# danijar/crafter

Measured on NVIDIA H100. Metric: env_steps_per_sec_random_policy, higher is better.
Workload: dtype int32/f64

## Files before the change

### crafter_b200/csrc/cr_kernels.h

```cpp
#pragma once
#include "cr_common.h"
#include "cr_geom.h"
#include "cr_noise.h"
#include "cr_render.h"
#include "cr_update.h"
#include "cr_worldgen.h"

#ifdef CR_SIMT
#define CR_DYN_SMEM(name) unsigned char *name = simt::dyn_smem()
#else
#define CR_DYN_SMEM(name) extern __shared__ __align__(16) unsigned char name[]
#endif

namespace cr {
namespace kernels {

#ifndef CR_UPDATE_WPB
#define CR_UPDATE_WPB 4
#endif
constexpr int UPDATE_WPB = CR_UPDATE_WPB;
constexpr int SEED_WPB = 4;
constexpr int RENDER_THREADS = RENDER_NT;
#ifndef CR_RENDER_MIN_CTAS
#define CR_RENDER_MIN_CTAS (RENDER_NT <= 128 ? 8 : DEF ? 4 : 2)
#endif
#ifndef CR_WG_THREADS
#define CR_WG_THREADS 256
#endif
#ifndef CR_WG_MIN_CTAS
#define CR_WG_MIN_CTAS 4
#endif
constexpr int WG_THREADS = CR_WG_THREADS;
#ifndef CR_OBJ_THREADS
#define CR_OBJ_THREADS 1024
#endif
constexpr int OBJ_THREADS = CR_OBJ_THREADS;
constexpr int INSTALL_THREADS = 256;

__host__ __device__ inline size_t align16(size_t v) { return (v + 15) & ~(size_t)15; }

__host__ __device__ inline size_t render_tile_offset(const Geom &g) {
  return align16(sizeof(RenderShared)) +
         (g.tile_cache ? align16((size_t)(N_TILES + 1) * g.ux * g.uy * sizeof(uint32_t)) : 16);
}

__host__ __device__ inline size_t update_smem_per_warp(const Geom &g) {
  return align16(sizeof(PlayerS)) + align16(sizeof(Ent) * ENT_SMEM) + align16(sizeof(uint32_t) * g.TW);
}

template <bool DEF>
__global__ void __launch_bounds__(UPDATE_WPB * 32)
k_update(Geom g, State st, const double *__restrict__ daylight, const int32_t *__restrict__ actions,
         float *reward, uint8_t *done, int auto_reset, int debug_skip) {
  geom_specialize<DEF>(g);
  CR_DYN_SMEM(smem);
  const int warp = threadIdx.x >> 5, lane = threadIdx.x & 31;
  const int env = blockIdx.x * UPDATE_WPB + warp;
  if (env >= g.B) return;
  unsigned char *base = smem + warp * update_smem_per_warp(g);
  PlayerS *P = reinterpret_cast<PlayerS *>(base);
  Ent *sents = reinterpret_cast<Ent *>(base + align16(sizeof(PlayerS)));
  uint32_t *stouched = reinterpret_cast<uint32_t *>(
      base + align16(sizeof(PlayerS)) + align16(sizeof(Ent) * ENT_SMEM));
  int action = actions[env];
  if (action < 0 || action >= N_ACTIONS) action = ACT_NOOP;
  const int kind = env_step(g, st, daylight, env, lane, action, P, sents, stouched, reward, done, auto_reset,
// ... 238 lines not shown
    wg_install_clear_rows(g, st, env, cx * CHUNK, imin(cx * CHUNK + CHUNK, g.W), threadIdx.x, INSTALL_THREADS);
    if (cx == 0)
      for (int c = threadIdx.x; c < g.TW; c += INSTALL_THREADS) st.touched[(size_t)env * g.TW + c] = 0;
    __syncthreads();
    if (g.incr_census)
      census_recount_column(g, st.mat + (size_t)env * g.NC, st.chunk_cnt + (size_t)env * g.NCH * 2, cx, threadIdx.x,
                            INSTALL_THREADS);
  }
}
template <bool DEF>
__global__ void __launch_bounds__(INSTALL_THREADS) k_install(Geom g, State st) {
  geom_specialize<DEF>(g);
  const int count = *st.reset_count;
  if (threadIdx.x == 0 && blockIdx.x < 1023) cr_stamp(4096 + (int)blockIdx.x, 4);
  for (int r = blockIdx.x; r < count; r += gridDim.x) {
    const int env = st.reset_list[r];
    wg_install_scatter(g, st, env, threadIdx.x, INSTALL_THREADS);
    if (threadIdx.x == 0) wg_install_player(g, st, env);
    __syncthreads();
  }
  if (threadIdx.x == 0 && blockIdx.x < 1023) cr_stamp(4096 + (int)blockIdx.x, 5);
}

__device__ __forceinline__ void store_tile(uint8_t *out, uint8_t *tile, size_t bytes, int tid, int evict_first) {
#ifndef CR_SIMT
  if ((bytes & 15) == 0) {
    asm volatile("fence.proxy.async.shared::cta;" ::: "memory");
    __syncthreads();
    if (tid == 0) {
      uint32_t saddr = (uint32_t)__cvta_generic_to_shared(tile);
      if (evict_first) {
        uint64_t policy;
        asm volatile("createpolicy.fractional.L2::evict_first.b64 %0, 1.0;" : "=l"(policy));
        asm volatile("cp.async.bulk.global.shared::cta.bulk_group.L2::cache_hint [%0], [%1], %2, %3;"
                     :: "l"(out), "r"(saddr), "r"((uint32_t)bytes), "l"(policy) : "memory");
      } else
      asm volatile("cp.async.bulk.global.shared::cta.bulk_group [%0], [%1], %2;"
                   :: "l"(out), "r"(saddr), "r"((uint32_t)bytes) : "memory");
      asm volatile("cp.async.bulk.commit_group;" ::: "memory");
      asm volatile("cp.async.bulk.wait_group.read 0;" ::: "memory");
    }
    return;
  }
#endif
  __syncthreads();
  for (size_t i = tid; i < bytes; i += RENDER_THREADS) out[i] = tile[i];
}

__global__ void __launch_bounds__(INSTALL_THREADS) k_recount(Geom g, State st) {
  for (int env = blockIdx.x; env < g.B; env += gridDim.x) {
    __syncthreads();
    census_recount(g, st.mat + (size_t)env * g.NC, st.chunk_cnt + (size_t)env * g.NCH * 2, threadIdx.x,
                   INSTALL_THREADS);
  }
}

template <bool DEF>
__device__ __forceinline__ void render_env(const Geom &g, const State &st, const RenderTables &rt, int env,
                                           uint8_t *out, int staged, unsigned char *smem, int tid, int use_view = 0) {
  RenderShared &S = *reinterpret_cast<RenderShared *>(smem);
  uint32_t *tiles = reinterpret_cast<uint32_t *>(smem + align16(sizeof(RenderShared)));
  uint8_t *tile = smem + render_tile_offset(g);
  const int trow = (tid & 31) == 0 && tid < 64 && env < 4096 ? (3 + (tid >> 5)) * 4096 + env : 1 << 30;
  cr_stamp(trow, 0);
  const int32_t *ps = st.pstate + (size_t)env * PS_COUNT;
  const double daylight = rt.daylight[imin(ps[PS_STEP], g.n_daylight - 1)];
  const size_t bytes = (size_t)g.sw * g.sh * 3;
  const RenderView *ahead = use_view ? reinterpret_cast<const RenderView *>(st.frame_view) + env : nullptr;
  render_stage(g, st, rt, env, tid, RENDER_THREADS, S, daylight, ahead, st.frame_night + env);
  cr_stamp(trow, 1);
  __syncthreads();
  cr_stamp(trow, 2);
  render_tiles(g, rt, S, tiles, tid, RENDER_THREADS, daylight < 0.5, ps[PS_SLEEPING]);
  cr_stamp(trow, 3);
  __syncthreads();
  cr_stamp(trow, 4);
  if (!DEF && !staged) {
    render_assemble(g, st, rt, S, tiles, env, tid, RENDER_THREADS, out, daylight, (bytes & 3) == 0);
    return;
  }
  render_assemble(g, st, rt, S, tiles, env, tid, RENDER_THREADS, tile, daylight, true, true);
  cr_stamp(trow, 5);
  store_tile(out, tile, bytes, tid, g.obs_evict_first);
  cr_stamp(trow, 6);
  cr_stamp(trow, 7, (daylight < 0.5 ? 1000 : 0) + S.V.n_jobs);
}

template <bool DEF>
__global__ void __launch_bounds__(RENDER_THREADS, CR_RENDER_MIN_CTAS)
k_render(Geom g, State st, RenderTables rt, uint8_t *__restrict__ obs, int staged,
         const int32_t *__restrict__ env_list, int out_by_env, int use_view) {
  geom_specialize<DEF>(g);
  CR_DYN_SMEM(smem);
  const int env = env_list ? env_list[blockIdx.x] : (int)blockIdx.x;
  const int row = out_by_env ? env : (int)blockIdx.x;
  render_env<DEF>(g, st, rt, env, obs + (size_t)row * g.sw * g.sh * 3, staged, smem, threadIdx.x, use_view);
}

constexpr int VIEW_WPB = 4;
template <bool DEF>
__global__ void __launch_bounds__(VIEW_WPB * 32) k_view(Geom g, State st, RenderTables rt) {
  geom_specialize<DEF>(g);
  __shared__ RenderView sv[VIEW_WPB];
  const int warp = threadIdx.x >> 5, lane = threadIdx.x & 31;
  const int env = blockIdx.x * VIEW_WPB + warp;
  if (threadIdx.x == 0 && blockIdx.x < 1024) cr_stamp(4096 + 3072 + (int)blockIdx.x, 0);
  if (env >= g.B || !(st.frame_night[env] & FRAME_FINAL)) return;
  RenderView &V = sv[warp];
  render_gather(g, st, rt, env, lane, V);
  __syncwarp();
  const Word16 *src = reinterpret_cast<const Word16 *>(&V);
  Word16 *dst = reinterpret_cast<Word16 *>(st.frame_view) + (size_t)env * VIEW_WORDS;
  for (int i = lane; i < VIEW_WORDS; i += 32) dst[i] = src[i];
  if (lane == 0 && blockIdx.x < 1024) cr_stamp(4096 + 3072 + (int)blockIdx.x, 1 + warp);
}

template <bool DEF>
__global__ void __launch_bounds__(RENDER_THREADS, 3)
k_terminal(Geom g, State st, RenderTables rt) {
// ... 35 lines not shown
```

### crafter_b200/csrc/cr_render.h

```cpp
#pragma once
#include "cr_common.h"

namespace cr {

#ifndef CR_MAX_OBJ_TILES
#define CR_MAX_OBJ_TILES 24
#endif
constexpr int MAX_OBJ_TILES = CR_MAX_OBJ_TILES;
constexpr int TILE_MAT0 = 0, TILE_OBJ0 = 13, TILE_ITEM0 = 13 + MAX_OBJ_TILES;
constexpr int N_TILES = TILE_ITEM0 + N_ITEMS;

struct RenderTables {
  const uint32_t *mat_tex;
  const uint32_t *obj_tex;
  const uint32_t *item_tile;
  const double *vignette;
  const double *daylight;
  const uint16_t *colx;
  const uint16_t *rowy;
};

struct alignas(16) RenderView {
  int32_t inv[N_ITEMS];
  int32_t n_obj, n_jobs, pad0, pad1;
// ... 65 lines not shown
CR_DEV void render_plan(const Geom &g, RenderView &V, int lane);

CR_DEV void render_tables(int tid, int nthreads, RenderShared &S, double daylight) {
  const double inv_d = 1 - daylight;
  for (int v = tid - CR_LANES; v < 256; v += nthreads - CR_LANES) {
    const double dv = (double)v;
    S.D[v] = dv;
    S.A[v] = daylight * dv;
    double half = (1 - 0.5) * dv;
    S.B[0][v] = inv_d * (half + 0.5 * 0.0);
    S.B[1][v] = inv_d * (half + 0.5 * 16.0);
    S.B[2][v] = inv_d * (half + 0.5 * 64.0);
    S.inv255[v] = (float)v / 255.0f;
  }
}

CR_DEV void render_gather(const Geom &g, const State &st, const RenderTables &rt, int env, int lane,
                          RenderView &V);

struct alignas(16) Word16 { uint64_t a, b; };
constexpr int VIEW_WORDS = (int)(sizeof(RenderView) / 16);

CR_DEV void render_stage(const Geom &g, const State &st, const RenderTables &rt, int env, int tid,
                         int nthreads, RenderShared &S, double daylight, const RenderView *ahead = nullptr,
                         const uint8_t *flag = nullptr) {
  if (tid >= CR_LANES) {
    render_tables(tid, nthreads, S, daylight);
  } else if (ahead) {
    constexpr int PER = (VIEW_WORDS + CR_LANES - 1) / CR_LANES;
    const Word16 *src = reinterpret_cast<const Word16 *>(ahead);
    Word16 *dst = reinterpret_cast<Word16 *>(&S.V);
    Word16 w[PER];
#pragma unroll
    for (int q = 0; q < PER; ++q) {
      const int i = tid + q * CR_LANES;
      if (i < VIEW_WORDS) w[q] = src[i];
    }
    if (*flag & FRAME_FINAL) {
#pragma unroll
      for (int q = 0; q < PER; ++q) {
        const int i = tid + q * CR_LANES;
        if (i < VIEW_WORDS) dst[i] = w[q];
      }
    } else {
      render_gather(g, st, rt, env, tid, S.V);
    }
  } else {
    render_gather(g, st, rt, env, tid, S.V);
  }
}

CR_DEV void render_gather(const Geom &g, const State &st, const RenderTables &rt, int env, int lane,
                          RenderView &V) {
  const int32_t *ps = st.pstate + (size_t)env * PS_COUNT;
  const int px = ps[PS_PX], py = ps[PS_PY], sleeping = ps[PS_SLEEPING];
  const uint8_t *mat = st.mat + (size_t)env * g.NC;
  const uint16_t *objmap = st.objmap + (size_t)env * g.NC;
  const Ent *ents = st.ents + (size_t)env * g.CAP;
  const int offx = g.gx / 2, offy = g.gy / 2;
  const int32_t *inv = st.inventory + (size_t)env * N_ITEMS;
  for (int i = lane; i < N_ITEMS; i += CR_LANES) V.inv[i] = inv[i];
  cr_syncwarp();
  constexpr int MAXC = 256 / CR_LANES > 8 ? 256 : 8;
  const int cells = g.vw * g.vh;
  int gcell[MAXC], mm[MAXC], slot[MAXC];
#pragma unroll
  for (int q = 0; q < MAXC; ++q) {
    const int c = lane + q * CR_LANES;
    gcell[q] = -1; mm[q] = 0; slot[q] = 0;
    if (c < cells) {
      const int i = c / g.vh, j = c - i * g.vh;
      const int wx = px + i - offx, wy = py + j - offy;
// ... 55 lines not shown
    }
    n += cr_popc(mask);
  }
  present = cr_reduce_or(present) & 0x1FFFu;
  const int n_mat = cr_popc(present), n_obj = imin(n, MAX_OBJ_TILES);
  for (int m = lane; m < 13; m += CR_LANES)
    if ((present >> m) & 1u) V.job_tile[cr_popc(present & ((1u << m) - 1u))] = (uint8_t)(TILE_MAT0 + m);
  for (int k = lane; k < n_obj; k += CR_LANES) V.job_tile[n_mat + k] = (uint8_t)(TILE_OBJ0 + k);
  int n_item = 0;
  for (int base = 0; base < N_ITEMS; base += CR_LANES) {
    const int i = base + lane;
    const bool has = i < N_ITEMS && V.inv[i] >= 1;
    const uint32_t mask = cr_ballot(has);
    if (has) V.job_tile[n_mat + n_obj + n_item + cr_popc(mask & cr_lanemask_lt(lane))] = (uint8_t)(TILE_ITEM0 + i);
    n_item += cr_popc(mask);
  }
  if (lane == 0) {
    V.job_tile[n_mat + n_obj + n_item] = (uint8_t)N_TILES;
    V.n_obj = n_obj;
    V.n_jobs = n_mat + n_obj + n_item + 1;
  }
}

CR_DEV void render_tiles(const Geom &g, const RenderTables &rt, const RenderShared &S, uint32_t *tiles,
                         int tid, int nthreads, bool dark, int sleeping) {
  const int tsz = g.ux * g.uy;
  const int n_jobs = S.V.n_jobs;
  int t = (int)mulhi32((uint32_t)tid, g.tsz_magic), texel = tid - t * tsz;
  const int sq = g.tile_sq, sr = g.tile_sr;
  (void)nthreads;
  while (t < n_jobs) {
    const int tile = S.V.job_tile[t];
    uint32_t color;
    bool fx = !dark;
    if (tile < TILE_OBJ0) {
      color = rt.mat_tex[tile * tsz + texel] & 0x00FFFFFFu;
    } else if (tile < TILE_ITEM0) {
      const int c = S.V.ocell[tile - TILE_OBJ0];
      color = blend_texel(S, rt.mat_tex[S.V.tmat[c] * tsz + texel], rt.obj_tex[S.V.tobj[c] * tsz + texel]);
    } else if (tile < N_TILES) {
      const int index = tile - TILE_ITEM0;
      int amount = S.V.inv[index];
      if (amount > 9) amount = 0;
      color = rt.item_tile[(index * 10 + amount) * tsz + texel] & 0x00FFFFFFu;
      fx = false;
    } else {
      color = 0;
      fx = false;
    }
    tiles[tile * tsz + texel] = fx ? color_fx(S, color, color, sleeping) : color;
    texel += sr; t += sq;
    if (texel >= tsz) { texel -= tsz; ++t; }
  }
}

struct RenderCtx {
  bool dark;
  int sleeping;
  double amount;
  uint32_t world_seed, step;
};

CR_DEV uint32_t night_pixel_v(const RenderShared &S, const RenderCtx &C, uint32_t c, double vignette,
                              uint32_t w) {
  const double u = (double)(int64_t)(((uint64_t)32 << 32) + (uint64_t)w * 95u) * (1.0 / 4294967296.0);
  const double mask = C.amount * vignette;
  const double om = 1 - mask, mu = mask * u;
  const int n0 = (int)(om * S.D[c & 0xFF] + mu);
  const int n1 = (int)(om * S.D[(c >> 8) & 0xFF] + mu);
  const int n2 = (int)(om * S.D[(c >> 16) & 0xFF] + mu);
  return color_mix3(S, c, n0, n1, n2);
}
CR_DEV uint32_t night_pixel_w(const Geom &g, const RenderTables &rt, const RenderShared &S,
                              const RenderCtx &C, uint32_t c, int cx, int cy, uint32_t w) {
  const uint32_t rgb = night_pixel_v(S, C, c, rt.vignette[cy * g.lw + cx], w);
  return C.sleeping ? sleep_fx(rgb) : rgb;
}
CR_DEV uint32_t night_pixel(const Geom &g, const RenderTables &rt, const RenderShared &S,
                            const RenderCtx &C, uint32_t c, int cx, int cy, U4 &nz, int &nz_block) {
  if ((cx >> 2) != nz_block) {
    nz = philox4x32(C.world_seed, D_NOISE, (uint32_t)(cx >> 2), C.step, (uint32_t)cy, 0);
    nz_block = cx >> 2;
  }
  return night_pixel_w(g, rt, S, C, c, cx, cy, nz.w[cx & 3]);
// ... 20 lines not shown
  } else {
    color = rt.mat_tex[S.V.tmat[cell] * tsz + texel] & 0x00FFFFFFu;
    if (S.V.tobj[cell] != 255) color = blend_texel(S, color, rt.obj_tex[S.V.tobj[cell] * tsz + texel]);
    if (!night) return color_fx(S, color, color, C.sleeping);
  }
  return night_pixel(g, rt, S, C, color, i * g.ux + tx, j * g.uy + ty, nz, nz_block);
}

CR_DEV void store_group(uint8_t *tile_out, int p, const uint32_t *px, int count, bool words_ok) {
  if (words_ok && count == 4) {
    uint32_t *w = (uint32_t *)(tile_out + (size_t)p * 3);
    w[0] = px[0] | (px[1] << 24);
    w[1] = (px[1] >> 8) | (px[2] << 16);
    w[2] = (px[2] >> 16) | (px[3] << 8);
  } else {
    for (int k = 0; k < count; ++k) {
      tile_out[(size_t)(p + k) * 3 + 0] = (uint8_t)px[k];
      tile_out[(size_t)(p + k) * 3 + 1] = (uint8_t)(px[k] >> 8);
      tile_out[(size_t)(p + k) * 3 + 2] = (uint8_t)(px[k] >> 16);
    }
  }
}

CR_DEV void render_assemble(const Geom &g, const State &st, const RenderTables &rt,
                            const RenderShared &S, const uint32_t *tiles, int env, int tid,
                            int nthreads, uint8_t *out, double daylight, bool words_ok, bool out_shared = false) {
  const int32_t *ps = st.pstate + (size_t)env * PS_COUNT;
  RenderCtx C;
  C.dark = daylight < 0.5;
  C.sleeping = ps[PS_SLEEPING];
  C.amount = 2 * (0.5 - daylight);
  C.world_seed = (uint32_t)ps[PS_WORLD_SEED];
  C.step = (uint32_t)ps[PS_STEP];
  const int tsz = g.ux * g.uy;
  if (g.g4_log2 >= 0 && nthreads == RENDER_NT && g.tile_cache) {
    const int gcol = tid & ((1 << g.g4_log2) - 1), band = tid >> g.g4_log2;
    const int y0 = band * g.band_rows, y1 = imin(g.sh, y0 + g.band_rows);
    const int black = N_TILES * tsz;
    int ci[4], toff[4], cx[4];
    bool colok[4];
#pragma unroll
    for (int k = 0; k < 4; ++k) {
      const uint32_t cxi = rt.colx[gcol * 4 + k];
      colok[k] = cxi != 0xFFFFu;
      ci[k] = colok[k] ? (int)(cxi >> 8) * g.vh : -1;
      toff[k] = colok[k] ? (int)(cxi & 0xFF) * g.uy : 0;
      cx[k] = colok[k] ? (int)(cxi >> 8) * g.ux + (int)(cxi & 0xFF) : 0;
    }
    const bool aligned4 = (g.bx & 3) == 0;
    const int out0 = gcol * 4;
    const bool any_col = colok[0] || colok[1] || colok[2] || colok[3];
#define CR_ROW_STATE()                   \
    int cur_j = -1, base[4] = {black, black, black, black};                                  \
    bool slow = false;
#define CR_ROW_LOOKUP()                                                                      \
        const int j = ryi >> 8, ty = ryi & 0xFF;                                             \
// ... 130 lines not shown
#undef CR_DAY_ROWS
#undef CR_NIGHT_ROWS
#undef CR_NIGHT_GROUP
#undef CR_DAY_RUNS
#undef CR_ROW_LOOKUP
#undef CR_ROW_SLOW
#undef CR_PIXEL
#undef CR_ROW_STORE
  } else {
    const int G = (g.sw + 3) >> 2;
    for (int q = tid; q < G * g.sh; q += nthreads) {
      const int y = q / G, x0 = (q - y * G) * 4;
      const uint32_t ryi = rt.rowy[y];
      const int count = imin(4, g.sw - x0);
      U4 nz; nz.w[0] = nz.w[1] = nz.w[2] = nz.w[3] = 0;
      int nz_block = -1;
      uint32_t px[4];
      for (int k = 0; k < count; ++k)
        px[k] = render_pixel(g, rt, S, tiles, C, rt.colx[x0 + k], ryi, nz, nz_block);
      store_group(out, y * g.sw + x0, px, count, words_ok && (((size_t)(y * g.sw + x0) * 3) & 3) == 0);
    }
  }
}

CR_DEV uint8_t semantic_cell(const Geom &g, const State &st, int env, int cell) {
  int slot = st.objmap[(size_t)env * g.NC + cell];
  if (slot) return (uint8_t)(12 + st.ents[(size_t)env * g.CAP + slot].type);
  return st.mat[(size_t)env * g.NC + cell] & 0x7F;
}

}
```

### crafter_b200/csrc/crafter_kernels.cu

```cuda
#include <cuda_runtime.h>
#include <stdio.h>
#include <stdlib.h>
#include <string.h>

#include <mutex>

#include "../../include/crafter_b200.h"
#include "cr_common.h"
#include "cr_geom.h"
#include "cr_noise.h"
#include "cr_render.h"
#include "cr_update.h"
#include "cr_worldgen.h"
#include "cr_kernels.h"

using namespace cr;
using namespace cr::kernels;

namespace {

#define CR_LAUNCH(KERNEL, DEFAULT, GRID, BLOCK, SMEM, STREAM, ...)                       \
  do {                                                                                   \
    if (DEFAULT) KERNEL<true><<<GRID, BLOCK, SMEM, STREAM>>>(__VA_ARGS__);               \
    else KERNEL<false><<<GRID, BLOCK, SMEM, STREAM>>>(__VA_ARGS__);                      \
// ... 24 lines not shown
  static int n = 0;
  std::lock_guard<std::mutex> lock(mu);
  int i = 0;
  while (i < n && funcs[i] != func) ++i;
  if (i == n) {
    if (n == 32) return cudaErrorInvalidValue;
    funcs[n] = func; have[n] = 0; ++n;
  }
  if (bytes <= have[i]) return cudaSuccess;
  cudaError_t e = cudaFuncSetAttribute(func, cudaFuncAttributeMaxDynamicSharedMemorySize, (int)bytes);
  if (e == cudaSuccess) have[i] = bytes;
  return e;
}

}

struct GraphSlot {
  cudaGraphExec_t exec;
  const void *actions, *obs, *reward, *done, *reward_host, *done_host;
  int kernels;
};

enum { TK_UPDATE = 0, TK_INSTALL, TK_RENDER, TK_SEED, TK_MAT, TK_OBJ, TK_AHEAD, TK_BALANCE, TK_COUNT };

struct cr_handle {
  int device;
  Geom g;
  State st;
  RenderTables rt;
  int auto_reset;
  int use_graph;
  int num_sms;
  size_t update_smem, render_smem, balance_smem, terminal_smem;
  int balance_threads;
  int render_staged;
  int64_t launches;
  cudaStream_t side, side2, side3;
  cudaEvent_t ev_fork, ev_join, ev_mat, ev_ahead, ev_inst, ev_d2h, ev_post, ev_bal, ev_view;
  int is_default;
  int timing;
  int debug_skip;
  cudaEvent_t t_ev[TK_COUNT][2];
  double t_ms[TK_COUNT];
  int64_t t_n;
  GraphSlot slots[2];
  float *d2h_reward;
  uint8_t *d2h_done;
  int32_t *err_word;
};

namespace {

inline void tmark(cr_handle *h, int id, int end, cudaStream_t s) {
  if (!h->timing) return;
  cudaStreamCaptureStatus cap = cudaStreamCaptureStatusNone;
  cudaStreamIsCapturing(s, &cap);
  if (cap == cudaStreamCaptureStatusActive) cudaEventRecordWithFlags(h->t_ev[id][end], s, cudaEventRecordExternal);
  else cudaEventRecord(h->t_ev[id][end], s);
// ... 36 lines not shown
  CR_LAUNCH(k_wg_mat, h->is_default, mat_grid, WG_THREADS, 0, s, g, h->st, list, count, only_invalid);
  tmark(h, TK_MAT, 1, s);
  int obj_grid = g.B < h->num_sms * 2 ? g.B : h->num_sms * 2;
  tmark(h, TK_OBJ, 0, s);
  CR_LAUNCH(k_wg_obj, h->is_default, obj_grid, OBJ_THREADS, 0, s, g, h->st, list, count, only_invalid);
  tmark(h, TK_OBJ, 1, s);
  if (ahead) CR_CUDA(cudaStreamWaitEvent(s, h->ev_ahead, 0));
  CR_CUDA(cudaGetLastError());
  return n;
}

int launch_install(cr_handle *h, cudaStream_t s) {
  int grid = h->g.B < h->num_sms * 8 ? h->g.B : h->num_sms * 8;
  long long parts = (long long)h->g.B * h->g.ncx;
  int map_grid = (int)(parts < (long long)h->num_sms * 8 ? parts : (long long)h->num_sms * 8);
  tmark(h, TK_INSTALL, 0, s);
  CR_LAUNCH(k_install_map, h->is_default, map_grid, INSTALL_THREADS, 0, s, h->g, h->st);
  CR_LAUNCH(k_install, h->is_default, grid, INSTALL_THREADS, 0, s, h->g, h->st);
  tmark(h, TK_INSTALL, 1, s);
  CR_CUDA(cudaGetLastError());
  return 2;
}

int launch_render(cr_handle *h, uint8_t *obs, cudaStream_t s, const int32_t *env_list = nullptr, int n_envs = -1,
                  int out_by_env = 0, int use_view = 0) {
  tmark(h, TK_RENDER, 0, s);
  CR_LAUNCH(k_render, h->is_default, n_envs < 0 ? h->g.B : n_envs, RENDER_THREADS, h->render_smem, s, h->g,
            h->st, h->rt, obs, h->render_staged, env_list, out_by_env, use_view);
  tmark(h, TK_RENDER, 1, s);
  CR_CUDA(cudaGetLastError());
  return 1;
}
int launch_render_and_prefetch(cr_handle *h, uint8_t *obs, cudaStream_t s, int seeded) {
  CR_CUDA(cudaEventRecord(h->ev_fork, s));
  CR_CUDA(cudaStreamWaitEvent(h->side, h->ev_fork, 0));
  int n = 0, k;
  if (obs) {
    if ((k = launch_render(h, obs, s)) < 0) return k;
    n += k;
  }
  if ((k = launch_worldgen(h, h->side, h->st.reset_list, h->st.reset_count, 0, 1, seeded)) < 0) return k;
  n += k;
  CR_CUDA(cudaEventRecord(h->ev_join, h->side));
  CR_CUDA(cudaStreamWaitEvent(s, h->ev_join, 0));
  return n;
}

int enqueue_d2h(cr_handle *h, const float *reward, const uint8_t *done, cudaStream_t s) {
  CR_CUDA(cudaMemcpyAsync(h->d2h_reward, reward, (size_t)h->g.B * sizeof(float), cudaMemcpyDeviceToHost, s));
  CR_CUDA(cudaMemcpyAsync(h->d2h_done, done, (size_t)h->g.B, cudaMemcpyDeviceToHost, s));
  return 0;
}

int enqueue_step(cr_handle *h, const int32_t *actions, uint8_t *obs, float *reward, uint8_t *done,
                 cudaStream_t s) {
  const Geom &g = h->g;
  const State &st = h->st;
  int n = 0, k;
#ifdef CR_MEMSET_FIRST
  CR_CUDA(cudaMemsetAsync(st.reset_count, 0, sizeof(int32_t), s));
  CR_CUDA(cudaMemsetAsync(st.balance_count, 0, sizeof(int32_t), s));
// ... 27 lines not shown
      n += 1;
    }
    if ((k = launch_install(h, h->side)) < 0) return k;
    n += k;
    CR_CUDA(cudaEventRecord(h->ev_inst, h->side));
    if ((k = launch_worldgen(h, h->side, st.reset_list, st.reset_count, 0, 1, 1)) < 0) return k;
    n += k;
    CR_CUDA(cudaMemsetAsync(st.reset_count, 0, sizeof(int32_t), h->side));
    CR_CUDA(cudaEventRecord(h->ev_join, h->side));
  }
  const int bal_ctas = g.B < h->num_sms * 4 ? g.B : h->num_sms * 4;
  tmark(h, TK_BALANCE, 0, s);
  CR_LAUNCH(k_post, h->is_default, bal_ctas + (st.frame_order ? 1 : 0), h->balance_threads, h->balance_smem, s, g, st,
            h->rt.daylight, bal_ctas);
  tmark(h, TK_BALANCE, 1, s);
  CR_CUDA(cudaGetLastError());
  n += 1;
  CR_CUDA(cudaEventRecord(h->ev_post, s));
  CR_CUDA(cudaStreamWaitEvent(h->side2, h->ev_post, 0));
  CR_CUDA(cudaMemsetAsync(st.balance_count, 0, sizeof(int32_t), h->side2));
  CR_CUDA(cudaEventRecord(h->ev_bal, h->side2));
  if (h->auto_reset) CR_CUDA(cudaStreamWaitEvent(s, h->ev_inst, 0));
  if (st.frame_view) CR_CUDA(cudaStreamWaitEvent(s, h->ev_view, 0));
  if ((k = launch_render(h, obs, s, st.frame_order, -1, 1, st.frame_view != nullptr)) < 0) return k;
  n += k;
  CR_CUDA(cudaStreamWaitEvent(s, h->ev_bal, 0));
  if (h->auto_reset) CR_CUDA(cudaStreamWaitEvent(s, h->ev_join, 0));
  if (d2h) CR_CUDA(cudaStreamWaitEvent(s, h->ev_d2h, 0));
  return n;
}

void destroy_handle(cr_handle *h) {
  if (!h) return;
  for (int i = 0; i < 2; ++i)
    if (h->slots[i].exec) cudaGraphExecDestroy(h->slots[i].exec);
  cudaStream_t streams[] = {h->side, h->side2, h->side3};
  for (cudaStream_t st : streams)
    if (st) { cudaStreamSynchronize(st); cudaStreamDestroy(st); }
  cudaEvent_t evs[] = {h->ev_mat, h->ev_ahead, h->ev_inst, h->ev_d2h, h->ev_fork, h->ev_join, h->ev_post, h->ev_bal,
                       h->ev_view};
  for (cudaEvent_t e : evs)
    if (e) cudaEventDestroy(e);
  for (int i = 0; i < TK_COUNT; ++i)
    for (int j = 0; j < 2; ++j)
      if (h->t_ev[i][j]) cudaEventDestroy(h->t_ev[i][j]);
  if (h->err_word) cudaFree(h->err_word);
  if (h->st.frame_order) cudaFree(h->st.frame_order);
  free(h);
}

bool env_is(const char *name, char c) {
  const char *v = getenv(name);
  return v && v[0] == c;
}

int create_on_device(cr_handle *h, const cr_config *c, const cr_tables *t, const cr_state *s) {
  Geom &g = h->g;
  if (const char *msg = geom_from_config(*c, g)) return fail_msg(msg);
  state_from_abi(*s, h->st);
  h->st.frame_order = nullptr; h->st.frame_night = nullptr; h->st.frame_view = nullptr;
  h->is_default = geom_is_default(g) && !env_is("CRAFTER_B200_NO_SPECIALIZE", '1');
  h->rt.mat_tex = t->mat_tex; h->rt.obj_tex = t->obj_tex; h->rt.item_tile = t->item_tile;
  h->rt.vignette = t->vignette; h->rt.daylight = t->daylight; h->rt.colx = t->colx;
  h->rt.rowy = t->rowy;
  h->auto_reset = c->auto_reset;
  const char *tm = getenv("CRAFTER_B200_TIMING");
  h->timing = tm && (tm[0] == '1' || tm[0] == '2') ? tm[0] - '0' : 0;
  const char *ds = getenv("CRAFTER_B200_DEBUG_SKIP");
  h->debug_skip = ds ? atoi(ds) : 0;
// ... 6 lines not shown
  CR_CUDA(cudaDeviceGetAttribute(&h->num_sms, cudaDevAttrMultiProcessorCount, dev));
  if (!env_is("CRAFTER_B200_FRAME_ORDER", '0')) {
    const size_t head = align16((size_t)g.B * (sizeof(int32_t) + 1));
    const size_t views = env_is("CRAFTER_B200_VIEW_AHEAD", '0') ? 0 : (size_t)g.B * sizeof(RenderView);
    CR_CUDA(cudaMalloc(&h->st.frame_order, head + views));
    CR_CUDA(cudaMemset(h->st.frame_order, 0, head + views));
    h->st.frame_night = reinterpret_cast<uint8_t *>(h->st.frame_order + g.B);
    if (views) h->st.frame_view = reinterpret_cast<unsigned char *>(h->st.frame_order) + head;
  }
  int max_smem = 0;
  CR_CUDA(cudaDeviceGetAttribute(&max_smem, cudaDevAttrMaxSharedMemoryPerBlockOptin, dev));
  h->update_smem = UPDATE_WPB * update_smem_per_warp(g);
  if (h->update_smem > (size_t)max_smem) return fail_msg("view too large for the update window");
  h->balance_smem = balance_smem(g);
  h->balance_threads = g.NCH * 3 > 4 * BALANCE_THREADS ? BALANCE_THREADS_MAX : BALANCE_THREADS;
  if (h->balance_smem > (size_t)max_smem) return fail_msg("area too large for k_balance");
  CR_CUDA(raise_smem((const void *)k_post<true>, h->balance_smem));
  CR_CUDA(raise_smem((const void *)k_post<false>, h->balance_smem));
  const size_t tile = align16((size_t)g.sw * g.sh * 3);
  if (g.tile_cache && render_tile_offset(g) > (size_t)max_smem) g.tile_cache = 0;
  const size_t fixed = render_tile_offset(g);
  if (fixed > (size_t)max_smem) return fail_msg("unit too large for the tile cache");
  h->render_staged = fixed + tile <= (size_t)max_smem / 2;
  h->render_smem = fixed + (h->render_staged ? tile : 0);
  if (!h->render_staged) h->is_default = 0;
  CR_CUDA(raise_smem((const void *)k_render<true>, h->render_smem));
  CR_CUDA(raise_smem((const void *)k_render<false>, h->render_smem));
  CR_CUDA(raise_smem((const void *)k_update<true>, h->update_smem));
  CR_CUDA(raise_smem((const void *)k_update<false>, h->update_smem));
  g.obs_evict_first = !env_is("CRAFTER_B200_OBS_EVICT_FIRST", '0');
  if (h->st.final_obs) {
    h->terminal_smem = terminal_smem(g, h->render_smem);
    if (!h->render_staged || !g.tile_cache || h->terminal_smem > (size_t)max_smem)
      return fail_msg("final_obs needs a frame that fits the shared-memory staging");
    CR_CUDA(raise_smem((const void *)k_terminal<true>, h->terminal_smem));
    CR_CUDA(raise_smem((const void *)k_terminal<false>, h->terminal_smem));
  }
  if (h->timing)
    for (int i = 0; i < TK_COUNT; ++i)
      for (int j = 0; j < 2; ++j) CR_CUDA(cudaEventCreate(&h->t_ev[i][j]));
  CR_CUDA(cudaStreamCreateWithFlags(&h->side, cudaStreamNonBlocking));
  CR_CUDA(cudaStreamCreateWithFlags(&h->side2, cudaStreamNonBlocking));
  CR_CUDA(cudaStreamCreateWithFlags(&h->side3, cudaStreamNonBlocking));
  cudaEvent_t *evs[] = {&h->ev_mat, &h->ev_ahead, &h->ev_inst, &h->ev_d2h, &h->ev_fork, &h->ev_join, &h->ev_post, &h->ev_bal,
                        &h->ev_view};
  for (cudaEvent_t *e : evs) CR_CUDA(cudaEventCreateWithFlags(e, cudaEventDisableTiming));
  return 0;
}

}

struct DeviceGuard {
  int prev = -1;
  explicit DeviceGuard(int want) {
    int cur = want;
// ... 91 lines not shown
                 uint8_t *done_host, int32_t *actions_dev, uint8_t *obs_dev, float *reward_dev,
                 uint8_t *done_dev, void *stream) {
  if (!h || !actions_host || !reward_host || !done_host) return fail_msg("null argument");
  DeviceGuard on_device(h->device);
  cudaStream_t s = (cudaStream_t)stream;
  const size_t B = (size_t)h->g.B;
  CR_CUDA(cudaMemcpyAsync(actions_dev, actions_host, B * sizeof(int32_t), cudaMemcpyHostToDevice, s));
  h->d2h_reward = reward_host;
  h->d2h_done = done_host;
  int rc = cr_step(h, actions_dev, obs_dev, reward_dev, done_dev, stream);
  h->d2h_reward = nullptr;
  h->d2h_done = nullptr;
  if (rc) return rc;
  if (obs_host)
    CR_CUDA(cudaMemcpyAsync(obs_host, obs_dev, B * h->g.sw * h->g.sh * 3, cudaMemcpyDeviceToHost, s));
  CR_CUDA(cudaStreamSynchronize(s));
  return 0;
}

int cr_render(cr_handle *h, uint8_t *obs, void *stream) {
  if (!h || !obs) return fail_msg("null argument");
  DeviceGuard on_device(h->device);
  const bool as_step = h->st.frame_view && env_is("CRAFTER_B200_RENDER_AS_STEP", '1');
  int k = as_step ? launch_render(h, obs, (cudaStream_t)stream, h->st.frame_order, -1, 1, 1)
                  : launch_render(h, obs, (cudaStream_t)stream);
  if (k < 0) return k;
  h->launches += k;
  return 0;
}

int cr_render_envs(cr_handle *h, const int32_t *env_ids, int n, uint8_t *obs, void *stream) {
  if (!h || !obs || !env_ids) return fail_msg("null argument");
  DeviceGuard on_device(h->device);
  if (n < 0 || n > h->g.B) return fail_msg("cr_render_envs: n out of range");
  if (n == 0) return 0;
  int k = launch_render(h, obs, (cudaStream_t)stream, env_ids, n);
  if (k < 0) return k;
  h->launches += k;
  return 0;
}

int cr_semantic(cr_handle *h, uint8_t *out, void *stream) {
  if (!h || !out) return fail_msg("null argument");
  DeviceGuard on_device(h->device);
  size_t n = (size_t)h->g.B * h->g.NC;
  k_semantic<<<(unsigned)((n + 255) / 256), 256, 0, (cudaStream_t)stream>>>(h->g, h->st, out);
  CR_CUDA(cudaGetLastError());
  h->launches += 1;
  return 0;
}

int cr_recount(cr_handle *h, void *stream) {
  if (!h) return fail_msg("null handle");
  if (!h->g.incr_census) return 0;
  DeviceGuard on_device(h->device);
  const int grid = h->g.B < h->num_sms * 8 ? h->g.B : h->num_sms * 8;
  k_recount<<<grid, INSTALL_THREADS, 0, (cudaStream_t)stream>>>(h->g, h->st);
  CR_CUDA(cudaGetLastError());
  h->launches += 1;
// ... 42 lines not shown
```

Measured before the change: 29.86 million.

## Make render kernel persistent with double-buffered staging and prefetched per-frame state

Turns k_render into a persistent kernel sized to resident CTAs that pulls frames from an atomic ticket counter. It prefetches the next frame's env id, player state, daylight and precomputed view with cp.async, and double-buffers the output staging tile so the bulk store of one frame overlaps assembly of the next. It also batches texture loads in render_tiles so several fetches are in flight at once. In exchange it uses more shared memory per CTA, which may cut occupancy, adds ticket atomics and reset logic, and makes the render loop harder to follow.

```diff
diff --git a/crafter_b200/csrc/cr_kernels.h b/crafter_b200/csrc/cr_kernels.h
--- a/crafter_b200/csrc/cr_kernels.h
+++ b/crafter_b200/csrc/cr_kernels.h
@@ -42,6 +42,9 @@
 __host__ __device__ inline size_t render_tile_offset(const Geom &g) {
   return align16(sizeof(RenderShared)) +
          (g.tile_cache ? align16((size_t)(N_TILES + 1) * g.ux * g.uy * sizeof(uint32_t)) : 16);
+}
+__host__ __device__ inline size_t render_smem_of(const Geom &g, int out_bufs) {
+  return render_tile_offset(g) + (size_t)out_bufs * align16((size_t)g.sw * g.sh * 3);
 }
 
 __host__ __device__ inline size_t update_smem_per_warp(const Geom &g) {
@@ -326,7 +329,7 @@
   if (threadIdx.x == 0 && blockIdx.x < 1023) cr_stamp(4096 + (int)blockIdx.x, 5);
 }
 
-__device__ __forceinline__ void store_tile(uint8_t *out, uint8_t *tile, size_t bytes, int tid, int evict_first) {
+__device__ __forceinline__ void store_tile_issue(uint8_t *out, uint8_t *tile, size_t bytes, int tid, int evict_first) {
 #ifndef CR_SIMT
   if ((bytes & 15) == 0) {
     asm volatile("fence.proxy.async.shared::cta;" ::: "memory");
@@ -342,7 +345,6 @@
       asm volatile("cp.async.bulk.global.shared::cta.bulk_group [%0], [%1], %2;"
                    :: "l"(out), "r"(saddr), "r"((uint32_t)bytes) : "memory");
       asm volatile("cp.async.bulk.commit_group;" ::: "memory");
-      asm volatile("cp.async.bulk.wait_group.read 0;" ::: "memory");
     }
     return;
   }
@@ -350,6 +352,32 @@
   __syncthreads();
   for (size_t i = tid; i < bytes; i += RENDER_THREADS) out[i] = tile[i];
 }
+__device__ __forceinline__ void bulk_wait_read(int pending) {
+#ifndef CR_SIMT
+  if (pending == 0) asm volatile("cp.async.bulk.wait_group.read 0;" ::: "memory");
+  else asm volatile("cp.async.bulk.wait_group.read 1;" ::: "memory");
+#else
+  (void)pending;
+#endif
+}
+__device__ __forceinline__ void store_tile(uint8_t *out, uint8_t *tile, size_t bytes, int tid, int evict_first) {
+  store_tile_issue(out, tile, bytes, tid, evict_first);
+  if (tid == 0) bulk_wait_read(0);
+}
+
+#ifdef CR_SIMT
+__device__ __forceinline__ void cr_cp_async4(void *dst, const void *src) { memcpy(dst, src, 4); }
+__device__ __forceinline__ void cr_cp_async16(void *dst, const void *src) { memcpy(dst, src, 16); }
+__device__ __forceinline__ void cr_cp_async_wait() {}
+#else
+__device__ __forceinline__ void cr_cp_async4(void *dst, const void *src) {
+  asm volatile("cp.async.ca.shared.global [%0], [%1], 4;" :: "r"(cr_saddr(dst)), "l"(src) : "memory");
+}
+__device__ __forceinline__ void cr_cp_async16(void *dst, const void *src) {
+  asm volatile("cp.async.cg.shared.global [%0], [%1], 16;" :: "r"(cr_saddr(dst)), "l"(src) : "memory");
+}
+__device__ __forceinline__ void cr_cp_async_wait() { asm volatile("cp.async.wait_all;" ::: "memory"); }
+#endif
 
 __global__ void __launch_bounds__(INSTALL_THREADS) k_recount(Geom g, State st) {
   for (int env = blockIdx.x; env < g.B; env += gridDim.x) {
@@ -361,7 +389,7 @@
 
 template <bool DEF>
 __device__ __forceinline__ void render_env(const Geom &g, const State &st, const RenderTables &rt, int env,
-                                           uint8_t *out, int staged, unsigned char *smem, int tid, int use_view = 0) {
+                                           uint8_t *out, int staged, unsigned char *smem, int tid) {
   RenderShared &S = *reinterpret_cast<RenderShared *>(smem);
   uint32_t *tiles = reinterpret_cast<uint32_t *>(smem + align16(sizeof(RenderShared)));
   uint8_t *tile = smem + render_tile_offset(g);
@@ -370,8 +398,7 @@
   const int32_t *ps = st.pstate + (size_t)env * PS_COUNT;
   const double daylight = rt.daylight[imin(ps[PS_STEP], g.n_daylight - 1)];
   const size_t bytes = (size_t)g.sw * g.sh * 3;
-  const RenderView *ahead = use_view ? reinterpret_cast<const RenderView *>(st.frame_view) + env : nullptr;
-  render_stage(g, st, rt, env, tid, RENDER_THREADS, S, daylight, ahead, st.frame_night + env);
+  render_stage(g, st, rt, env, tid, RENDER_THREADS, S, daylight);
   cr_stamp(trow, 1);
   __syncthreads();
   cr_stamp(trow, 2);
@@ -390,15 +417,120 @@
   cr_stamp(trow, 7, (daylight < 0.5 ? 1000 : 0) + S.V.n_jobs);
 }
 
+struct alignas(16) FrameSlot {
+  int32_t ps[PS_COUNT];
+  int32_t frame, env;
+  uint32_t flags_word;
+  int32_t pad;
+  double daylight;
+  double pad2;
+};
+
 template <bool DEF>
 __global__ void __launch_bounds__(RENDER_THREADS, CR_RENDER_MIN_CTAS)
 k_render(Geom g, State st, RenderTables rt, uint8_t *__restrict__ obs, int staged,
-         const int32_t *__restrict__ env_list, int out_by_env, int use_view) {
+         const int32_t *__restrict__ env_list, int out_by_env, int use_view, int n_frames = -1, int out_bufs = 1,
+         int32_t *ticket = nullptr) {
   geom_specialize<DEF>(g);
   CR_DYN_SMEM(smem);
-  const int env = env_list ? env_list[blockIdx.x] : (int)blockIdx.x;
-  const int row = out_by_env ? env : (int)blockIdx.x;
-  render_env<DEF>(g, st, rt, env, obs + (size_t)row * g.sw * g.sh * 3, staged, smem, threadIdx.x, use_view);
+  __shared__ FrameSlot slots[2];
+  __shared__ RenderView vnext_s;
+  if (n_frames < 0) n_frames = g.B;
+  RenderShared &S = *reinterpret_cast<RenderShared *>(smem);
+  uint32_t *tiles = reinterpret_cast<uint32_t *>(smem + align16(sizeof(RenderShared)));
+  RenderView *vnext = &vnext_s;
+  uint8_t *staging = smem + render_tile_offset(g);
+  const int tid = threadIdx.x, lane = tid & 31;
+  const size_t bytes = (size_t)g.sw * g.sh * 3;
+  auto fetch_env = [&](FrameSlot &F, int frame) {
+    F.frame = frame;
+    if (frame < n_frames) {
+      if (env_list) cr_cp_async4(&F.env, env_list + frame);
+      else F.env = frame;
+    }
+  };
+  auto fetch_state = [&](FrameSlot &F) {
+    if (F.frame >= n_frames) return;
+    const int env = F.env;
+    if (lane < PS_COUNT) cr_cp_async4(&F.ps[lane], st.pstate + (size_t)env * PS_COUNT + lane);
+    if (use_view) {
+      if (lane == PS_COUNT) cr_cp_async4(&F.flags_word, st.frame_night + (env & ~3));
+      const Word16 *src = reinterpret_cast<const Word16 *>(st.frame_view) + (size_t)env * VIEW_WORDS;
+      for (int i = lane; i < VIEW_WORDS; i += 32) cr_cp_async16(reinterpret_cast<Word16 *>(vnext) + i, src + i);
+    }
+  };
+  auto fetch_daylight = [&](FrameSlot &F) {
+    if (F.frame < n_frames) F.daylight = rt.daylight[imin(F.ps[PS_STEP], g.n_daylight - 1)];
+  };
+  if (tid < 32) {
+    if (lane == 0) fetch_env(slots[0], (int)blockIdx.x);
+    cr_cp_async_wait();
+    __syncwarp();
+    fetch_state(slots[0]);
+    cr_cp_async_wait();
+    __syncwarp();
+    if (lane == 0) fetch_daylight(slots[0]);
+  }
+  __syncthreads();
+  int next_frame = 0;
+  for (int k = 0;; ++k) {
+    FrameSlot &F = slots[k & 1], &Fn = slots[(k + 1) & 1];
+    if (F.frame >= n_frames) break;
+    const int env = F.env;
+    const double daylight = F.daylight;
+    uint8_t *out = obs + (size_t)(out_by_env ? env : F.frame) * bytes;
+    const int trow = (tid & 31) == 0 && tid < 64 && env < 4096 ? (3 + (tid >> 5)) * 4096 + env : 1 << 30;
+    cr_stamp(trow, 0);
+    if (tid >= CR_LANES) {
+      render_tables(tid, RENDER_THREADS, S, daylight);
+    } else {
+      if (lane == 0) next_frame = (int)gridDim.x + (ticket ? atomicAdd(ticket, 1) : F.frame);
+      if (use_view && ((F.flags_word >> (8 * (env & 3))) & FRAME_FINAL)) {
+        const Word16 *src = reinterpret_cast<const Word16 *>(vnext);
+        Word16 *dst = reinterpret_cast<Word16 *>(&S.V);
+        for (int i = lane; i < VIEW_WORDS; i += 32) dst[i] = src[i];
+      } else {
+        render_gather(g, st, rt, env, lane, S.V);
+      }
+    }
+    cr_stamp(trow, 1);
+    __syncthreads();
+    cr_stamp(trow, 2);
+    if (tid == 0) fetch_env(Fn, next_frame);
+    render_tiles(g, rt, S, tiles, tid, RENDER_THREADS, daylight < 0.5, F.ps[PS_SLEEPING]);
+    cr_stamp(trow, 3);
+    const bool direct = !DEF && !staged;
+    uint8_t *tile = staging + (size_t)(out_bufs > 1 ? (k & 1) : 0) * align16(bytes);
+    if (tid == 0 && !direct) bulk_wait_read(out_bufs > 1 ? 1 : 0);
+    __syncthreads();
+    cr_stamp(trow, 4);
+    if (tid < 32) {
+      cr_cp_async_wait();
+      __syncwarp();
+      fetch_state(Fn);
+    }
+    const RenderCtx C = render_ctx(F.ps, daylight);
+    render_assemble(g, rt, S, tiles, C, tid, RENDER_THREADS, direct ? out : tile, direct ? (bytes & 3) == 0 : true,
+                    !direct);
+    cr_stamp(trow, 5);
+    cr_stamp(trow, 7, (long long)(blockIdx.x + 1) * 10000 + (daylight < 0.5 ? 1000 : 0) + S.V.n_jobs);
+    if (tid < 32) {
+      cr_cp_async_wait();
+      __syncwarp();
+      if (lane == 0) fetch_daylight(Fn);
+    }
+    if (direct) __syncthreads();
+    else store_tile_issue(out, tile, bytes, tid, g.obs_evict_first);
+    cr_stamp(trow, 6);
+  }
+  if (tid == 0) {
+    bulk_wait_read(0);
+    __threadfence();
+    if (ticket && atomicAdd(ticket + 1, 1) == (int)gridDim.x - 1) {
+      ticket[0] = 0;
+      ticket[1] = 0;
+    }
+  }
 }
 
 constexpr int VIEW_WPB = 4;
diff --git a/crafter_b200/csrc/cr_render.h b/crafter_b200/csrc/cr_render.h
--- a/crafter_b200/csrc/cr_render.h
+++ b/crafter_b200/csrc/cr_render.h
@@ -111,32 +111,9 @@
 constexpr int VIEW_WORDS = (int)(sizeof(RenderView) / 16);
 
 CR_DEV void render_stage(const Geom &g, const State &st, const RenderTables &rt, int env, int tid,
-                         int nthreads, RenderShared &S, double daylight, const RenderView *ahead = nullptr,
-                         const uint8_t *flag = nullptr) {
-  if (tid >= CR_LANES) {
-    render_tables(tid, nthreads, S, daylight);
-  } else if (ahead) {
-    constexpr int PER = (VIEW_WORDS + CR_LANES - 1) / CR_LANES;
-    const Word16 *src = reinterpret_cast<const Word16 *>(ahead);
-    Word16 *dst = reinterpret_cast<Word16 *>(&S.V);
-    Word16 w[PER];
-#pragma unroll
-    for (int q = 0; q < PER; ++q) {
-      const int i = tid + q * CR_LANES;
-      if (i < VIEW_WORDS) w[q] = src[i];
-    }
-    if (*flag & FRAME_FINAL) {
-#pragma unroll
-      for (int q = 0; q < PER; ++q) {
-        const int i = tid + q * CR_LANES;
-        if (i < VIEW_WORDS) dst[i] = w[q];
-      }
-    } else {
-      render_gather(g, st, rt, env, tid, S.V);
-    }
-  } else {
-    render_gather(g, st, rt, env, tid, S.V);
-  }
+                         int nthreads, RenderShared &S, double daylight) {
+  if (tid >= CR_LANES) render_tables(tid, nthreads, S, daylight);
+  else render_gather(g, st, rt, env, tid, S.V);
 }
 
 CR_DEV void render_gather(const Geom &g, const State &st, const RenderTables &rt, int env, int lane,
@@ -238,6 +215,7 @@
   }
 }
 
+constexpr int TILE_BATCH = 4;
 CR_DEV void render_tiles(const Geom &g, const RenderTables &rt, const RenderShared &S, uint32_t *tiles,
                          int tid, int nthreads, bool dark, int sleeping) {
   const int tsz = g.ux * g.uy;
@@ -246,27 +224,46 @@
   const int sq = g.tile_sq, sr = g.tile_sr;
   (void)nthreads;
   while (t < n_jobs) {
-    const int tile = S.V.job_tile[t];
-    uint32_t color;
-    bool fx = !dark;
-    if (tile < TILE_OBJ0) {
-      color = rt.mat_tex[tile * tsz + texel] & 0x00FFFFFFu;
-    } else if (tile < TILE_ITEM0) {
-      const int c = S.V.ocell[tile - TILE_OBJ0];
-      color = blend_texel(S, rt.mat_tex[S.V.tmat[c] * tsz + texel], rt.obj_tex[S.V.tobj[c] * tsz + texel]);
-    } else if (tile < N_TILES) {
-      const int index = tile - TILE_ITEM0;
-      int amount = S.V.inv[index];
-      if (amount > 9) amount = 0;
-      color = rt.item_tile[(index * 10 + amount) * tsz + texel] & 0x00FFFFFFu;
-      fx = false;
-    } else {
-      color = 0;
-      fx = false;
-    }
-    tiles[tile * tsz + texel] = fx ? color_fx(S, color, color, sleeping) : color;
-    texel += sr; t += sq;
-    if (texel >= tsz) { texel -= tsz; ++t; }
+    int tl[TILE_BATCH], tx[TILE_BATCH];
+    uint32_t base[TILE_BATCH], tex[TILE_BATCH];
+#pragma unroll
+    for (int b = 0; b < TILE_BATCH; ++b) {
+      tl[b] = t < n_jobs ? S.V.job_tile[t] : -1;
+      tx[b] = texel;
+      base[b] = 0; tex[b] = 0;
+      const int tile = tl[b];
+      if (tile < 0 || tile >= N_TILES) {
+      } else if (tile < TILE_OBJ0) {
+        base[b] = rt.mat_tex[tile * tsz + texel];
+      } else if (tile < TILE_ITEM0) {
+        const int c = S.V.ocell[tile - TILE_OBJ0];
+        base[b] = rt.mat_tex[S.V.tmat[c] * tsz + texel];
+        tex[b] = rt.obj_tex[S.V.tobj[c] * tsz + texel];
+      } else {
+        const int index = tile - TILE_ITEM0;
+        int amount = S.V.inv[index];
+        if (amount > 9) amount = 0;
+        base[b] = rt.item_tile[(index * 10 + amount) * tsz + texel];
+      }
+      texel += sr; t += sq;
+      if (texel >= tsz) { texel -= tsz; ++t; }
+    }
+#pragma unroll
+    for (int b = 0; b < TILE_BATCH; ++b) {
+      const int tile = tl[b];
+      if (tile < 0) break;
+      uint32_t color;
+      bool fx = !dark;
+      if (tile < TILE_OBJ0) {
+        color = base[b] & 0x00FFFFFFu;
+      } else if (tile < TILE_ITEM0) {
+        color = blend_texel(S, base[b], tex[b]);
+      } else {
+        color = base[b] & 0x00FFFFFFu;
+        fx = false;
+      }
+      tiles[tile * tsz + tx[b]] = fx ? color_fx(S, color, color, sleeping) : color;
+    }
   }
 }
 
@@ -276,6 +273,15 @@
   double amount;
   uint32_t world_seed, step;
 };
+CR_DEV RenderCtx render_ctx(const int32_t *ps, double daylight) {
+  RenderCtx C;
+  C.dark = daylight < 0.5;
+  C.sleeping = ps[PS_SLEEPING];
+  C.amount = 2 * (0.5 - daylight);
+  C.world_seed = (uint32_t)ps[PS_WORLD_SEED];
+  C.step = (uint32_t)ps[PS_STEP];
+  return C;
+}
 
 CR_DEV uint32_t night_pixel_v(const RenderShared &S, const RenderCtx &C, uint32_t c, double vignette,
                               uint32_t w) {
@@ -342,16 +348,9 @@
   }
 }
 
-CR_DEV void render_assemble(const Geom &g, const State &st, const RenderTables &rt,
-                            const RenderShared &S, const uint32_t *tiles, int env, int tid,
-                            int nthreads, uint8_t *out, double daylight, bool words_ok, bool out_shared = false) {
-  const int32_t *ps = st.pstate + (size_t)env * PS_COUNT;
-  RenderCtx C;
-  C.dark = daylight < 0.5;
-  C.sleeping = ps[PS_SLEEPING];
-  C.amount = 2 * (0.5 - daylight);
-  C.world_seed = (uint32_t)ps[PS_WORLD_SEED];
-  C.step = (uint32_t)ps[PS_STEP];
+CR_DEV void render_assemble(const Geom &g, const RenderTables &rt, const RenderShared &S, const uint32_t *tiles,
+                            const RenderCtx &C, int tid, int nthreads, uint8_t *out, bool words_ok,
+                            bool out_shared = false) {
   const int tsz = g.ux * g.uy;
   if (g.g4_log2 >= 0 && nthreads == RENDER_NT && g.tile_cache) {
     const int gcol = tid & ((1 << g.g4_log2) - 1), band = tid >> g.g4_log2;
@@ -528,6 +527,12 @@
     }
   }
 }
+CR_DEV void render_assemble(const Geom &g, const State &st, const RenderTables &rt,
+                            const RenderShared &S, const uint32_t *tiles, int env, int tid,
+                            int nthreads, uint8_t *out, double daylight, bool words_ok, bool out_shared = false) {
+  const RenderCtx C = render_ctx(st.pstate + (size_t)env * PS_COUNT, daylight);
+  render_assemble(g, rt, S, tiles, C, tid, nthreads, out, words_ok, out_shared);
+}
 
 CR_DEV uint8_t semantic_cell(const Geom &g, const State &st, int env, int cell) {
   int slot = st.objmap[(size_t)env * g.NC + cell];
diff --git a/crafter_b200/csrc/crafter_kernels.cu b/crafter_b200/csrc/crafter_kernels.cu
--- a/crafter_b200/csrc/crafter_kernels.cu
+++ b/crafter_b200/csrc/crafter_kernels.cu
@@ -70,6 +70,7 @@
 };
 
 enum { TK_UPDATE = 0, TK_INSTALL, TK_RENDER, TK_SEED, TK_MAT, TK_OBJ, TK_AHEAD, TK_BALANCE, TK_COUNT };
+enum { RS_STEP = 0, RS_RENDER, RS_ENVS, RS_COUNT };
 
 struct cr_handle {
   int device;
@@ -82,6 +83,9 @@
   size_t update_smem, render_smem, balance_smem, terminal_smem;
   int balance_threads;
   int render_staged;
+  int render_bufs;
+  int render_ctas;
+  int32_t *render_tickets;
   int64_t launches;
   cudaStream_t side, side2, side3;
   cudaEvent_t ev_fork, ev_join, ev_mat, ev_ahead, ev_inst, ev_d2h, ev_post, ev_bal, ev_view;
@@ -164,11 +168,14 @@
   return 2;
 }
 
-int launch_render(cr_handle *h, uint8_t *obs, cudaStream_t s, const int32_t *env_list = nullptr, int n_envs = -1,
-                  int out_by_env = 0, int use_view = 0) {
+int launch_render(cr_handle *h, uint8_t *obs, cudaStream_t s, int site, const int32_t *env_list = nullptr,
+                  int n_envs = -1, int out_by_env = 0, int use_view = 0) {
+  const int n = n_envs < 0 ? h->g.B : n_envs;
+  const long long resident = (long long)h->num_sms * h->render_ctas;
+  const int grid = (int)(n < resident ? n : resident);
   tmark(h, TK_RENDER, 0, s);
-  CR_LAUNCH(k_render, h->is_default, n_envs < 0 ? h->g.B : n_envs, RENDER_THREADS, h->render_smem, s, h->g,
-            h->st, h->rt, obs, h->render_staged, env_list, out_by_env, use_view);
+  CR_LAUNCH(k_render, h->is_default, grid, RENDER_THREADS, h->render_smem, s, h->g, h->st, h->rt, obs,
+            h->render_staged, env_list, out_by_env, use_view, n, h->render_bufs, h->render_tickets + 2 * site);
   tmark(h, TK_RENDER, 1, s);
   CR_CUDA(cudaGetLastError());
   return 1;
@@ -178,7 +185,7 @@
   CR_CUDA(cudaStreamWaitEvent(h->side, h->ev_fork, 0));
   int n = 0, k;
   if (obs) {
-    if ((k = launch_render(h, obs, s)) < 0) return k;
+    if ((k = launch_render(h, obs, s, RS_RENDER)) < 0) return k;
     n += k;
   }
   if ((k = launch_worldgen(h, h->side, h->st.reset_list, h->st.reset_count, 0, 1, seeded)) < 0) return k;
@@ -252,7 +259,7 @@
   CR_CUDA(cudaEventRecord(h->ev_bal, h->side2));
   if (h->auto_reset) CR_CUDA(cudaStreamWaitEvent(s, h->ev_inst, 0));
   if (st.frame_view) CR_CUDA(cudaStreamWaitEvent(s, h->ev_view, 0));
-  if ((k = launch_render(h, obs, s, st.frame_order, -1, 1, st.frame_view != nullptr)) < 0) return k;
+  if ((k = launch_render(h, obs, s, RS_STEP, st.frame_order, -1, 1, st.frame_view != nullptr)) < 0) return k;
   n += k;
   CR_CUDA(cudaStreamWaitEvent(s, h->ev_bal, 0));
   if (h->auto_reset) CR_CUDA(cudaStreamWaitEvent(s, h->ev_join, 0));
@@ -275,6 +282,7 @@
     for (int j = 0; j < 2; ++j)
       if (h->t_ev[i][j]) cudaEventDestroy(h->t_ev[i][j]);
   if (h->err_word) cudaFree(h->err_word);
+  if (h->render_tickets) cudaFree(h->render_tickets);
   if (h->st.frame_order) cudaFree(h->st.frame_order);
   free(h);
 }
@@ -327,15 +335,32 @@
   const size_t fixed = render_tile_offset(g);
   if (fixed > (size_t)max_smem) return fail_msg("unit too large for the tile cache");
   h->render_staged = fixed + tile <= (size_t)max_smem / 2;
-  h->render_smem = fixed + (h->render_staged ? tile : 0);
   if (!h->render_staged) h->is_default = 0;
-  CR_CUDA(raise_smem((const void *)k_render<true>, h->render_smem));
-  CR_CUDA(raise_smem((const void *)k_render<false>, h->render_smem));
+  const void *render_fn = h->is_default ? (const void *)k_render<true> : (const void *)k_render<false>;
+  auto resident = [&](size_t smem, int *ctas) -> cudaError_t {
+    cudaError_t e = raise_smem((const void *)k_render<true>, smem);
+    if (e == cudaSuccess) e = raise_smem((const void *)k_render<false>, smem);
+    if (e == cudaSuccess) e = cudaOccupancyMaxActiveBlocksPerMultiprocessor(ctas, render_fn, RENDER_THREADS, smem);
+    return e;
+  };
+  h->render_bufs = h->render_staged ? 1 : 0;
+  h->render_smem = render_smem_of(g, h->render_bufs);
+  CR_CUDA(resident(h->render_smem, &h->render_ctas));
+  int two = 0;
+  if (h->render_staged && resident(render_smem_of(g, 2), &two) == cudaSuccess && two >= h->render_ctas) {
+    h->render_bufs = 2;
+    h->render_smem = render_smem_of(g, 2);
+    h->render_ctas = two;
+  }
+  cudaGetLastError();
+  if (h->render_ctas < 1) return fail_msg("k_render: no CTA fits an SM");
+  CR_CUDA(cudaMalloc(&h->render_tickets, RS_COUNT * 2 * sizeof(int32_t)));
+  CR_CUDA(cudaMemset(h->render_tickets, 0, RS_COUNT * 2 * sizeof(int32_t)));
   CR_CUDA(raise_smem((const void *)k_update<true>, h->update_smem));
   CR_CUDA(raise_smem((const void *)k_update<false>, h->update_smem));
   g.obs_evict_first = !env_is("CRAFTER_B200_OBS_EVICT_FIRST", '0');
   if (h->st.final_obs) {
-    h->terminal_smem = terminal_smem(g, h->render_smem);
+    h->terminal_smem = terminal_smem(g, fixed + tile);
     if (!h->render_staged || !g.tile_cache || h->terminal_smem > (size_t)max_smem)
       return fail_msg("final_obs needs a frame that fits the shared-memory staging");
     CR_CUDA(raise_smem((const void *)k_terminal<true>, h->terminal_smem));
@@ -473,8 +498,8 @@
   if (!h || !obs) return fail_msg("null argument");
   DeviceGuard on_device(h->device);
   const bool as_step = h->st.frame_view && env_is("CRAFTER_B200_RENDER_AS_STEP", '1');
-  int k = as_step ? launch_render(h, obs, (cudaStream_t)stream, h->st.frame_order, -1, 1, 1)
-                  : launch_render(h, obs, (cudaStream_t)stream);
+  int k = as_step ? launch_render(h, obs, (cudaStream_t)stream, RS_RENDER, h->st.frame_order, -1, 1, 1)
+                  : launch_render(h, obs, (cudaStream_t)stream, RS_RENDER);
   if (k < 0) return k;
   h->launches += k;
   return 0;
@@ -485,7 +510,7 @@
   DeviceGuard on_device(h->device);
   if (n < 0 || n > h->g.B) return fail_msg("cr_render_envs: n out of range");
   if (n == 0) return 0;
-  int k = launch_render(h, obs, (cudaStream_t)stream, env_ids, n);
+  int k = launch_render(h, obs, (cudaStream_t)stream, RS_ENVS, env_ids, n);
   if (k < 0) return k;
   h->launches += k;
   return 0;
```

New measurement: 30.58 million, median of 6. 1.02x the previous value.
